# swesterfeld/audiowmark

Hardware: AMD Instinct MI355X
Metric: audio seconds watermarked+decoded per wall-second (xRT), 44.1 kHz stereo (higher is better)
Workload: dtype f32; 1 GPU; 60 min stereo 44.1 kHz white noise per GPU resident in HBM, add+get incl. payload decode, payload 0123456789abcdef0011223344556677, strength 10; parallelism=1 GPU, patterns=108, payload_matches=104, ranks_seen=1

## Files before the change

audiowmark_amd/binding.py:

```python
import ctypes as C
import os

import numpy as np

_HERE = os.path.dirname(os.path.abspath(__file__))
N_BANDS = 81
BLOCK_FRAMES = 2226
SOFT_BITS = 858


class AwmError(RuntimeError):
    pass


def library_path():
    return os.path.join(_HERE, "libawm_hip.so")




def _load_hip_runtime():
    candidates = []
    try:
        import torch
# ... 61 lines not shown
lib.awm_version.restype = C.c_char_p
lib.awm_ctx_stream.restype = C.c_void_p
lib.awm_search_approx_d.restype = C.c_long
lib.awm_set_params.argtypes = [C.c_double, C.c_int, C.c_int, C.c_int, C.c_double, C.c_int, C.c_double]
lib.awm_set_params.restype = None
lib.awm_ctx_create.argtypes = [C.c_int, C.POINTER(_vp)]
lib.awm_ctx_destroy.argtypes = [_vp]
lib.awm_ctx_destroy.restype = None
lib.awm_ctx_synchronize.argtypes = [_vp]
lib.awm_ctx_stream.argtypes = [_vp]
lib.awm_ctx_set_stream.argtypes = [_vp, _vp]
lib.awm_stft_d.argtypes = [_vp, _vp, C.c_size_t, C.c_int, C.c_size_t, C.c_size_t, C.c_size_t, _vp]
lib.awm_add_init_block_max_d.argtypes = [_vp, _vp, C.c_size_t]
lib.awm_add_mix_d.argtypes = [_vp, _vp, _vp, C.c_size_t, C.c_int, _vp, C.c_double, C.c_size_t, _vp, _vp, _vp,
                              C.c_size_t, C.c_size_t]
lib.awm_add_limit_d.argtypes = [_vp, _vp, C.c_size_t, C.c_int, C.c_size_t, _vp, C.c_size_t, C.c_size_t]
lib.awm_add_d.argtypes = [_vp, _vp, _vp, C.c_size_t, C.c_int, _vp, C.c_double, C.c_int]
lib.awm_sync_fft_d.argtypes = [_vp, _vp, C.c_size_t, C.c_int, C.c_size_t, C.c_size_t, _vp, C.c_size_t, C.c_size_t, _vp, _vp]
lib.awm_sync_search_d.argtypes = [_vp, _vp, _vp, C.c_size_t, C.c_int, C.c_int, C.c_size_t, _vp, _vp, _vp]
lib.awm_search_approx_d.argtypes = [_vp, _vp, _vp, C.c_size_t, C.c_int, C.c_int, C.c_size_t, _vp, _vp, _vp]
lib.awm_block_soft_bits_d.argtypes = [_vp, _vp, _vp, C.c_size_t, C.c_int, _vp, C.c_size_t, _vp, _vp]
lib.awm_viterbi_decode.argtypes = [_vp, C.c_int, _vp, C.c_size_t, C.c_size_t, _vp, _vp]
lib.awm_add_watermark_d.argtypes = [_vp, _vp, C.c_char_p, _vp, _vp, C.c_size_t, C.c_int, C.c_int]
lib.awm_get_watermark_d.argtypes = [_vp, _vp, _vp, C.c_size_t, C.c_int, C.c_size_t, _vp]
lib.awm_add_get_watermark_d.argtypes = [_vp, _vp, C.c_char_p, _vp, _vp, C.c_size_t, C.c_int, C.c_int, C.c_size_t, _vp]
lib.awm_resample_frames.argtypes = [_vp, C.c_size_t, C.c_int, C.c_int]
lib.awm_resample_frames.restype = C.c_size_t
lib.awm_resample_d.argtypes = [_vp, _vp, C.c_size_t, C.c_int, C.c_int, C.c_int, _vp, C.c_size_t]
lib.awm_add_watermark_payloads_d.argtypes = [_vp, _vp, _vp, C.c_size_t, _vp, _vp, C.c_size_t, C.c_int, C.c_int]
lib.awm_debug_set_add_payloads_fused.argtypes = [C.c_int]
lib.awm_debug_set_add_payloads_fused.restype = None
lib.awm_debug_add_payloads_fused_in_use.argtypes = []
lib.awm_debug_add_payloads_fused_in_use.restype = C.c_int
lib.awm_debug_add_payloads_tile.argtypes = []
lib.awm_debug_add_payloads_tile.restype = C.c_int
lib.awm_add_watermark_batch_d.argtypes = [_vp, _vp, C.c_char_p, C.c_size_t, _vp, _vp, _vp, C.c_int]
lib.awm_get_watermark_batch_d.argtypes = [_vp, _vp, C.c_size_t, _vp, _vp, C.c_int, C.c_int, C.c_size_t, _vp, _vp]
lib.awm_add_watermark_batch_keys_d.argtypes = [_vp, _vp, C.c_char_p, C.c_size_t, _vp, _vp, _vp, C.c_int]
lib.awm_get_watermark_batch_keys_d.argtypes = [_vp, _vp, C.c_size_t, _vp, _vp, C.c_int, C.c_int, C.c_size_t, _vp, _vp]
lib.awm_decode_chunk_d.argtypes = [_vp, _vp, _vp, C.c_size_t, C.c_int, C.c_int, C.c_size_t, _vp]
lib.awm_tab_up_down.argtypes = [_vp, C.c_int, C.c_int, _vp, _vp]
lib.awm_tab_bit_pos.argtypes = [_vp, _vp]
lib.awm_tab_mix_entries.argtypes = [_vp, _vp]
lib.awm_tab_bit_order.argtypes = [_vp, C.c_size_t, _vp]
lib.awm_tab_frame_mod.argtypes = [_vp, C.c_char_p, _vp]
lib.awm_tab_sync_bits.argtypes = [_vp, C.c_int, _vp]
lib.awm_tab_window.argtypes = [C.c_size_t, _vp]
lib.awm_tab_synth_window.argtypes = [_vp]
lib.awm_conv_encode.argtypes = [C.c_int, _vp, C.c_size_t, _vp]
lib.awm_test_gen_noise.argtypes = [_vp, C.c_size_t, _vp]


class RawFormat(C.Structure):
    _fields_ = [("n_channels", C.c_int), ("sample_rate", C.c_int), ("bit_depth", C.c_int), ("encoding", C.c_int), ("big_endian", C.c_int)]


lib.awm_add_watermark_file.argtypes = [_vp, _vp, C.c_char_p, C.c_char_p, C.c_char_p, C.POINTER(RawFormat), C.POINTER(RawFormat)]
lib.awm_add_stream_watermark_file.argtypes = [_vp, _vp, C.c_char_p, C.c_char_p, C.c_char_p, C.POINTER(RawFormat), C.POINTER(RawFormat), C.c_size_t]
lib.awm_add_stream_create_at.argtypes = [_vp, _vp, C.c_char_p, C.c_int, C.c_size_t, C.c_size_t, C.POINTER(_vp)]
lib.awm_debug_sync_db_sliding_d.argtypes = [_vp, _vp, C.c_size_t, C.c_int, _vp, C.c_size_t, C.c_int, C.c_int, _vp]
lib.awm_get_watermark_file.argtypes = [_vp, _vp, C.c_char_p, C.POINTER(RawFormat), C.c_size_t, _vp]
lib.awm_add_get_watermark_file.argtypes = [_vp, _vp, C.c_char_p, C.c_char_p, C.c_char_p, C.POINTER(RawFormat), C.POINTER(RawFormat), C.c_size_t, _vp]
lib.awm_add_stream_create.argtypes = [_vp, _vp, C.c_char_p, C.c_int, C.c_size_t, C.POINTER(_vp)]
lib.awm_add_stream_destroy.argtypes = [_vp]
lib.awm_add_stream_destroy.restype = None
lib.awm_add_stream_input.argtypes = [_vp]
# ... 862 lines not shown
```

audiowmark_amd/csrc/hip/kernels.hh:

```
#pragma once
#include <hip/hip_runtime.h>
#include <cstddef>
#include <cstdint>

#if defined(__HIP_DEVICE_COMPILE__) && !defined(__gfx950__)
#error "audiowmark_amd's HIP kernels are written for gfx950 (MI355X) only"
#endif

namespace awmk {

struct DevTables
{
  const float2 *tw512;
  const float2 *tw1024;
  const float  *window;
  const float  *synth;
  const double2 *slide;
  const double2 *tw512d;
  const float2 *slide32;
};

hipError_t launch_stft_full (hipStream_t st, const DevTables& t, const float *pcm, int n_channels,
                             long long start_index, long long hop, long long frame_count, float2 *out);

// ... 86 lines not shown
struct SyncDbArgs
{
  const float *pcm;
  long long    n_frames;
  int          n_channels;
  int          per_channel;
  long long    base0, base_stride;
  const long long *stream_base;
  int          count0;
  const int   *stream_count;
  long long    n_streams;
  long long    hop;
  float       *out;
  long long    out_stream_stride;
  long long    ld;
  char        *have;
  long long    have_stream_stride;
  long long    first, last;
  int          tile_frames;
  int          xcd_interleave = 0;
  const int           *row_perm = nullptr;
  const unsigned char *band_pos = nullptr;
  int                  rows_per_plane = 0;
  float               *tail = nullptr;
  long long            tail_stream_stride = 0;
  int                  tables_per_slice = 0;
  int                  streams_per_slice = 0;
  long long            slice_stride = 0;
  const long long     *stream_range = nullptr;
  const int           *range_index = nullptr;
  int                  range_div = 1;
  int                  silent_frames_are_zero = 0;
  int                  skip_unread_silent_tiles = 0;
};
hipError_t launch_sync_db (hipStream_t st, const DevTables& t, const SyncDbArgs& a);
hipError_t launch_sync_db_sliding (hipStream_t st, const DevTables& t, const SyncDbArgs& a);
bool sliding_rows_have_tail (int n_channels);

struct SyncTableDev
{
  const int *packed;
  int        rows_per_bit;
  const unsigned *chains = nullptr;
  long long       chains_slice_stride = 0;
  int             planes_per_slice = 1;
  const int      *row_frames = nullptr;
};
void pack_scan_chains (const int *packed, int rows_per_bit, unsigned *out );
struct SyncScanArgs
{
  const float *db;
  const char  *have;
  int          have_is_run = 0;
  long long    plane_stride;
  long long    have_plane_stride;
  long long    row_stride, band_stride, have_row_stride;
  long long    n_lanes;
  const int   *lane_count;
  long long    n_planes;
  double       min_delta;
  double      *quality;
  long long    q_stride;
  SyncTableDev table;
};
hipError_t launch_sync_scan (hipStream_t st, const SyncScanArgs& a);
hipError_t launch_sync_scan_window (hipStream_t st, const SyncScanArgs& a, int total_frames);

struct GatheredScanArgs
// ... 18 lines not shown
};
constexpr size_t GATHERED_SCRATCH_BYTES_PER_PLANE = 18 * 128 * 4;
hipError_t launch_sync_scan_gathered (hipStream_t st, const GatheredScanArgs& a);

hipError_t launch_local_mean (hipStream_t st, const double *q, long long q_stride, long long n_start_frames,
                              double *raw_sorted, double *local_mean, int n_slices = 1);

struct PeakOut { long long p; double raw, mean; };
hipError_t launch_peak_select (hipStream_t st, const double *raw_sorted, const double *local_mean, long long n, double threshold,
                               unsigned int *count, PeakOut *out, unsigned int cap);
hipError_t launch_peak_select_slices (hipStream_t st, const double *raw_sorted, const double *local_mean, long long n, double threshold,
                                      unsigned int *count, int count_stride, PeakOut *out, unsigned int cap, int n_slices);

hipError_t launch_peak_topk (hipStream_t st, const PeakOut *in, const unsigned int *count, unsigned int cap, PeakOut *out, int k, int n_slices);
hipError_t launch_peak_topk_lists (hipStream_t st, const PeakOut *in, const unsigned int *count, int count_stride, unsigned int cap,
                                   PeakOut *out, int k, int n_slices, int n_lists);

struct SoftBitsArgs
{
  const float   *db;
  long long      block_stride, ld;
  int            n_channels;
  const int16_t *mix_frame;
  const uint8_t *mix_up, *mix_down;
  int            n_data_frames;
  int            frames_per_bit;
  int            block_frames;
  long long      n_blocks;
  float         *out;
  const int     *block_slice = nullptr;
  const long long *block_base = nullptr;
  const long long *stream_range = nullptr;
  const int       *range_index = nullptr;
};
hipError_t launch_soft_bits (hipStream_t st, const SoftBitsArgs& a);

struct SoftJobDev
{
  int       mode;
  int       n_src, src_off;
  int       len;
  int       norm0, norm1;
  long long out_off;
  int       order_off;
  int       pad;
};
struct SoftPrepArgs
{
  const float      *raw;
  int               n_bits;
  const int        *inv_order;
  const SoftJobDev *jobs;
  const int2       *src;
  long long         n_jobs;
  int               hard;
  float            *out;
};
hipError_t launch_soft_prep (hipStream_t st, const SoftPrepArgs& a);

hipError_t launch_viterbi (hipStream_t st, const float *const soft[3], const long long n_blocks[3], long long n_steps,
                           unsigned char *const decisions_ws[3], int *const bits_out[3], float *const error_out[3], unsigned int *sync_ws);
size_t viterbi_workspace_bytes (long long coded_len, int rate, long long n_blocks);
bool viterbi_steps_supported (long long n_steps);
size_t viterbi_sync_bytes (long long n_blocks);
double probe_dependent_launch_us (hipStream_t st);
const char *viterbi_form_description();
// ... 103 lines not shown
```

audiowmark_amd/csrc/hip/kernels.hip:

```cpp
#include "kernels.hh"
#include "awm_fft.hip.h"
#include <cstdlib>
#include <algorithm>
#include <type_traits>

namespace awmk {

constexpr int NB = 81;
constexpr int MIN_BAND = 20;
constexpr int WAVES = 4;

typedef const int __attribute__ ((address_space (4))) *const_int_ptr;

__device__ __forceinline__ void
load_shared_tables (const DevTables& t, float2 *s_tw, float *s_win, float2 *s_twb)
{
  fft512_load_twiddles (t.tw512, s_tw);
  for (int i = threadIdx.x; i < 1024; i += blockDim.x)
    s_win[i] = t.window[i];
  if (s_twb)
    for (int i = threadIdx.x; i < NB; i += blockDim.x)
      s_twb[i] = t.tw1024[MIN_BAND + i];
}


__device__ __forceinline__ void
fetch_stereo (const float *pcm, long long idx, int avail, int lane, float (&l)[16], float (&r)[16])
{
  const float *p = pcm + idx * 2;
  if (avail >= 1024 && ((reinterpret_cast<uintptr_t> (p) & 15) == 0))
    {
      const float4 *p4 = reinterpret_cast<const float4 *> (p);
#pragma unroll
      for (int j = 0; j < 8; j++)
        {
          const float4 v = p4[lane + 64 * j];
          l[2 * j] = v.x; r[2 * j] = v.y; l[2 * j + 1] = v.z; r[2 * j + 1] = v.w;
// ... 1604 lines not shown

hipError_t
launch_mix_max (hipStream_t st, const float *orig, const float *wm, float *out, long long n_frames, int n_channels,
                unsigned int *block_max, long long n_blocks, int limiter_block)
{
  const long long n_values = n_frames * n_channels;
  if (n_values <= 0)
    return hipSuccess;
  if ((long long) limiter_block * n_channels < MIX_RUN)
    return hipErrorInvalidValue;
  hipLaunchKernelGGL (mix_max_kernel, dim3 (unsigned ((n_values + MIX_RUN - 1) / MIX_RUN)), dim3 (256), 0, st, orig, wm, out, n_values,
                      n_channels, block_max, n_blocks, limiter_block);
  return hipGetLastError();
}

__global__ void
fill_u32_kernel (unsigned int *p, unsigned int v, size_t n)
{
  const size_t i = (size_t) blockIdx.x * blockDim.x + threadIdx.x;
  if (i < n)
    p[i] = v;
}
hipError_t
launch_fill_u32 (hipStream_t st, unsigned int *p, unsigned int v, size_t n)
{
  if (!n)
    return hipSuccess;
  hipLaunchKernelGGL (fill_u32_kernel, dim3 (unsigned ((n + 255) / 256)), dim3 (256), 0, st, p, v, n);
  return hipGetLastError();
}


__device__ __forceinline__ long long
sync_stream_base (const SyncDbArgs& a, long long stream)
{
  if (a.stream_base)
    return a.stream_base[stream];
  if (a.streams_per_slice > 0)
    return a.base0 + (stream % a.streams_per_slice) * a.base_stride + (stream / a.streams_per_slice) * a.slice_stride;
  return a.base0 + stream * a.base_stride;
}

__device__ __forceinline__ void
sync_stream_range (const SyncDbArgs& a, long long stream, long long& first, long long& last)
{
  first = a.first;
  last = a.last;
  if (a.stream_range)
    {
      const long long g = stream / a.range_div;
      const long long slice = a.range_index ? a.range_index[g] : g;
      first = a.stream_range[2 * slice];
      last = a.stream_range[2 * slice + 1];
      if (first < 0)
        first = last = 0x7fffffffffffffffLL;
    }
}


template<int CV, bool SPLIT, int TLD> __global__ void __launch_bounds__ (64 * WAVES)
sync_db_kernel (DevTables t, SyncDbArgs a)
{
  constexpr int TILE_LD = TLD, TILE_MAX = TLD - 1, SPLIT_COLS = TILE_MAX / 2;
  __shared__ float2 s_tw[512];
  __shared__ float  s_win[1024];
  __shared__ float2 s_twb[NB];
  __shared__ float2 s_x[WAVES][XBUF_ELEMS];
  __shared__ float  s_tile[NB * TILE_LD];
  __shared__ char   s_have[TILE_MAX];
  const int lane = threadIdx.x & 63, wave = threadIdx.x >> 6;
  if (a.silent_frames_are_zero && a.skip_unread_silent_tiles)
    {
      long long stream = blockIdx.y, tile_idx = blockIdx.x;
      if (a.xcd_interleave)
        {
          const long long j = blockIdx.x >> 3;
          stream = j % a.n_streams;
          tile_idx = (j / a.n_streams) * 8 + (blockIdx.x & 7);
        }
      const long long base = sync_stream_base (a, stream);
      const int count = a.stream_count ? a.stream_count[stream] : a.count0;
      long long sil_first, sil_last;
      sync_stream_range (a, stream, sil_first, sil_last);
      const long long tile0 = tile_idx * a.tile_frames;
      if (tile0 >= count)
        return;
      const long long n_here = (count - tile0) < a.tile_frames ? count - tile0 : a.tile_frames;
      const long long idx_before = base + (tile0 - 2) * a.hop, idx_after = base + (tile0 + n_here + 1) * a.hop;
      const int C = a.n_channels;
      if ((idx_after + 1024) * C < sil_first || idx_before * C > sil_last)
        return;
    }
  load_shared_tables (t, s_tw, s_win, s_twb);
  __syncthreads();

  long long stream = blockIdx.y, tile_idx = blockIdx.x;
  if (a.xcd_interleave)
    {
      const long long j = blockIdx.x >> 3;
      stream = j % a.n_streams;
      tile_idx = (j / a.n_streams) * 8 + (blockIdx.x & 7);
    }
  const int plane_ch = blockIdx.z;
  const long long base = sync_stream_base (a, stream);
  const int count = a.stream_count ? a.stream_count[stream] : a.count0;
  long long sil_first, sil_last;
  sync_stream_range (a, stream, sil_first, sil_last);
  const int TF = a.tile_frames;
  const long long tile0 = tile_idx * TF;
  if (tile0 >= count)
    return;
  const int C = a.n_channels;
  float2 *xbuf = s_x[wave];
  const int n_here = (count - tile0) < TF ? int (count - tile0) : TF;

  for (int ff = wave; ff < n_here; ff += WAVES)
    {
      const long long idx = base + (tile0 + ff) * a.hop;
      const long long f_first = idx * C, f_last = (idx + 1024) * C;
      const bool outside = idx < 0 || idx + 1024 > a.n_frames;
      const bool skip = (f_last < sil_first) || (f_first > sil_last) || outside;
      float acc0 = 0.f, acc1 = 0.f;
      float split0 = 0.f, split1 = 0.f;
      if (!skip)
        {
          if (CV == 2)
            {
              float in[2][16];
              fetch_stereo (a.pcm, idx, 1024, lane, in[0], in[1]);
              float2 za[8], zb[8];
              window_pack (in[0], s_win, lane, za);
              window_pack (in[1], s_win, lane, zb);
              fft512_forward2 (za, zb, xbuf, s_tw, lane);
              const int k0 = MIN_BAND + lane, k1 = MIN_BAND + 64 + lane;
              const bool second = lane < NB - 64;
              float2 pa[4], pb[4];
              lds_st (&xbuf[0 * 64 + lane], za[0]);
              lds_st (&xbuf[1 * 64 + lane], za[1]);
              lds_st (&xbuf[6 * 64 + lane], za[6]);
              lds_st (&xbuf[7 * 64 + lane], za[7]);
              wave_sync();
              pa[0] = lds_ld (&xbuf[zpos (k0)]);
              pa[1] = lds_ld (&xbuf[zpos (512 - k0)]);
              pa[2] = lds_ld (&xbuf[zpos (second ? k1 : k0)]);
              pa[3] = lds_ld (&xbuf[zpos (512 - (second ? k1 : k0))]);
              wave_sync();
              lds_st (&xbuf[0 * 64 + lane], zb[0]);
              lds_st (&xbuf[1 * 64 + lane], zb[1]);
// ... 52 lines not shown
          const float zero_db = db_from_complex (make_float2 (0.f, 0.f));
          const int n_ch = CV == 2 ? 2 : (a.per_channel ? 1 : C);
          for (int c = 0; c < n_ch; c++)
            {
              if (SPLIT && c == 1)
                {
                  split0 = acc0;
                  split1 = acc1;
                  acc0 = acc1 = 0.f;
                }
              acc0 = __fadd_rn (acc0, zero_db);
              acc1 = __fadd_rn (acc1, zero_db);
            }
        }
      if (SPLIT)
        {
          s_tile[lane * TILE_LD + ff] = split0;
          s_tile[lane * TILE_LD + SPLIT_COLS + ff] = acc0;
          if (lane < NB - 64)
            {
              s_tile[(64 + lane) * TILE_LD + ff] = split1;
              s_tile[(64 + lane) * TILE_LD + SPLIT_COLS + ff] = acc1;
            }
        }
      else
        {
          s_tile[lane * TILE_LD + ff] = acc0;
          if (lane < NB - 64)
            s_tile[(64 + lane) * TILE_LD + ff] = acc1;
        }
      if (lane == 0)
        s_have[ff] = skip ? 0 : 1;
    }
  __syncthreads();
  if (SPLIT)
    {
      for (int p = 0; p < 2; p++)
        {
          float *out = a.out + stream * a.out_stream_stride + (long long) p * NB * a.ld + tile0;
          for (int i = threadIdx.x; i < NB * n_here; i += blockDim.x)
            {
              const int band = i / n_here, ff = i - band * n_here;
              out[band * a.ld + ff] = s_tile[band * TILE_LD + p * SPLIT_COLS + ff];
            }
        }
    }
  else
    {
      const long long plane = a.per_channel ? plane_ch : 0;
      float *out = a.out + stream * a.out_stream_stride + plane * NB * a.ld + tile0;
      for (int i = threadIdx.x; i < NB * n_here; i += blockDim.x)
        {
          const int band = i / n_here, ff = i - band * n_here;
          out[band * a.ld + ff] = s_tile[band * TILE_LD + ff];
        }
    }
  if (a.have && plane_ch == 0)
    for (int i = threadIdx.x; i < n_here; i += blockDim.x)
      a.have[stream * a.have_stream_stride + tile0 + i] = s_have[i];
}

hipError_t
launch_sync_db (hipStream_t st, const DevTables& t, const SyncDbArgs& a)
{
  if (a.n_streams <= 0 || a.tile_frames <= 0 || a.tile_frames > 72)
    return a.n_streams <= 0 ? hipSuccess : hipErrorInvalidValue;
  int max_count = a.count0;
  if (max_count <= 0)
    return hipSuccess;
  const unsigned tiles = unsigned ((max_count + a.tile_frames - 1) / a.tile_frames);
  if (a.n_streams > 65535LL * 1)
    {
      SyncDbArgs b = a;
      long long done = 0;
      while (done < a.n_streams)
        {
          const long long n = (a.n_streams - done) > 65535 ? 65535 : (a.n_streams - done);
          b.n_streams = n;
          b.base0 = a.base0 + done * a.base_stride;
          b.stream_base = a.stream_base ? a.stream_base + done : nullptr;
          b.stream_count = a.stream_count ? a.stream_count + done : nullptr;
          b.out = a.out + done * a.out_stream_stride;
          b.have = a.have ? a.have + done * a.have_stream_stride : nullptr;
          hipError_t e = launch_sync_db (st, t, b);
          if (e != hipSuccess)
            return e;
          done += n;
        }
      return hipSuccess;
    }
  const bool small = a.tile_frames <= 32;
  if (a.n_channels == 2 && a.per_channel)
    {
      SyncDbArgs b = a;
      b.tile_frames = 16;
      const unsigned split_tiles = unsigned ((max_count + b.tile_frames - 1) / b.tile_frames);
      hipLaunchKernelGGL ((sync_db_kernel<2, true, 33>), dim3 (split_tiles, unsigned (a.n_streams), 1), dim3 (64 * WAVES), 0, st, t, b);
      return hipGetLastError();
    }
  const unsigned planes = a.per_channel ? unsigned (a.n_channels) : 1u;
  dim3 grid (tiles, unsigned (a.n_streams), planes);
  SyncDbArgs b = a;
  if (!a.stream_base && !a.stream_count && a.n_streams >= 2 && a.n_streams <= 8 && planes == 1)
    {
      b.xcd_interleave = 1;
      grid = dim3 (unsigned (((tiles + 7) / 8) * 8 * a.n_streams), 1, 1);
    }
  if (a.n_channels == 2 && !a.per_channel)
    {
      if (small)
        hipLaunchKernelGGL ((sync_db_kernel<2, false, 33>), grid, dim3 (64 * WAVES), 0, st, t, b);
      else
        hipLaunchKernelGGL ((sync_db_kernel<2, false, 73>), grid, dim3 (64 * WAVES), 0, st, t, b);
    }
  else
    {
      if (small)
        hipLaunchKernelGGL ((sync_db_kernel<1, false, 33>), grid, dim3 (64 * WAVES), 0, st, t, b);
      else
        hipLaunchKernelGGL ((sync_db_kernel<1, false, 73>), grid, dim3 (64 * WAVES), 0, st, t, b);
    }
  return hipGetLastError();
}

constexpr int SL_TILE = 16;

__device__ __forceinline__ double
dpp_from_lower_lane (double v)
{
  const int lo = __builtin_amdgcn_update_dpp (0, __double2loint (v), 0x138, 0xf, 0xf, true);
  const int hi = __builtin_amdgcn_update_dpp (0, __double2hiint (v), 0x138, 0xf, 0xf, true);
  return __hiloint2double (hi, lo);
}
__device__ __forceinline__ double
dpp_from_upper_lane (double v)
{
  const int lo = __builtin_amdgcn_update_dpp (0, __double2loint (v), 0x130, 0xf, 0xf, true);
  const int hi = __builtin_amdgcn_update_dpp (0, __double2hiint (v), 0x130, 0xf, 0xf, true);
  return __hiloint2double (hi, lo);
}

__device__ __forceinline__ long long
wave_uniform (long long v)
{
  const int lo = __builtin_amdgcn_readfirstlane (int (v)), hi = __builtin_amdgcn_readfirstlane (int (v >> 32));
  return (long long) (((unsigned long long) (unsigned int) hi << 32) | (unsigned int) lo);
}

typedef __attribute__ ((address_space (1))) float global_float;
__device__ __forceinline__ global_float *
uniform_global (const float *p)
{
  return (global_float *) (unsigned long long) wave_uniform ((long long) (unsigned long long) p);
}

template<int CV> __global__ void __launch_bounds__ (64 * WAVES) __attribute__ ((amdgpu_waves_per_eu (3, 3)))
sync_db_sliding_kernel (DevTables t, SyncDbArgs a)
{
  constexpr int SCRATCH_FLOATS = XBUF_ELEMS * 4 > NB * SL_TILE ? XBUF_ELEMS * 4 : NB * SL_TILE;
  __shared__ __attribute__ ((aligned (16))) float s_scratch[WAVES][SCRATCH_FLOATS];
  __shared__ unsigned char s_pos[WAVES][NB + 3];
  __shared__ __attribute__ ((aligned (16))) double s_delta[WAVES][SL_TILE * 8 * CV];
  __shared__ int s_nzd[WAVES][SL_TILE * CV];
  __shared__ int s_x0[WAVES][SL_TILE * CV];
  {
    const int w = threadIdx.x >> 6, l = threadIdx.x & 63;
    const long long s = (long long) blockIdx.x * WAVES + w;
    const long long tslice = (a.tables_per_slice && s < a.n_streams) ? (a.range_index ? a.range_index[s / a.range_div] : s / a.range_div) : 0;
    for (int b = l; b < NB; b += 64)
      s_pos[w][b] = (a.band_pos && s < a.n_streams) ? a.band_pos[(tslice * a.rows_per_plane + s % a.rows_per_plane) * NB + b] : (unsigned char) b;
  }
  __syncthreads();

  const int lane = threadIdx.x & 63, wave = threadIdx.x >> 6;
  const long long stream = (long long) blockIdx.x * WAVES + wave;
  if (stream >= a.n_streams)
    return;
  const long long perm_slice = a.tables_per_slice ? (a.range_index ? a.range_index[stream / a.range_div] : stream / a.range_div) : 0;
  const long long out_slot = wave_uniform (a.row_perm ? (stream / a.rows_per_plane) * a.rows_per_plane
// ... 1136 lines not shown
  const int n_bits = a.n_data_frames / a.frames_per_bit;
  if (bit >= n_bits)
    return;
  const float *db = a.db + blk * a.block_stride;
  const int C = a.n_channels;
  const long long mix0 = a.block_slice ? (long long) a.block_slice[blk] * a.n_data_frames * 30 : 0;
  const int16_t *mix_frame = a.mix_frame + mix0;
  const uint8_t *mix_up = a.mix_up + mix0, *mix_down = a.mix_down + mix0;
  double umag = 0, dmag = 0;
  for (int f = bit * a.frames_per_bit; f < (bit + 1) * a.frames_per_bit; f++)
    for (int ch = 0; ch < C; ch++)
      {
        const float *plane = db + (long long) ch * NB * a.ld;
        for (int j = 0; j < 30; j++)
          {
            const int b = f * 30 + j;
            const int frame = mix_frame[b];
            const int next = frame + 1 < a.block_frames ? frame + 1 : frame - 1;
            const int prev = frame - 1 >= 0 ? frame - 1 : frame + 1;
            const float *pu = plane + (long long) (mix_up[b] - MIN_BAND) * a.ld;
            const float *pd = plane + (long long) (mix_down[b] - MIN_BAND) * a.ld;
            umag += pu[frame];
            umag -= double (__fadd_rn (pu[prev], pu[next])) * 0.5;
            dmag += pd[frame];
            dmag -= double (__fadd_rn (pd[prev], pd[next])) * 0.5;
          }
      }
  a.out[blk * n_bits + bit] = float (umag - dmag);
}

constexpr int SB_WAVES = 4;
constexpr int SB_BPW = 4;
constexpr int SB_MAX_ITEMS = 256;

__global__ void __launch_bounds__ (64 * SB_WAVES)
soft_bits_wave_kernel (SoftBitsArgs a, int groups_per_block)
{
  extern __shared__ __attribute__ ((aligned (16))) float4 s_item_dyn[];
  const int lane = threadIdx.x & 63, wave = threadIdx.x >> 6;
  const long long slot = blockIdx.x >> 3;
  const long long blk = (slot / groups_per_block) * 8 + (blockIdx.x & 7);
  const int group = int (slot % groups_per_block);
  if (blk >= a.n_blocks)
    return;
  const int n_bits = a.n_data_frames / a.frames_per_bit;
  const int bit0 = (group * SB_WAVES + wave) * SB_BPW;
  if (bit0 >= n_bits)
    return;
  const float *db = a.db + blk * a.block_stride;
  const int C = a.n_channels;
  const long long mix0 = a.block_slice ? (long long) a.block_slice[blk] * a.n_data_frames * 30 : 0;
  const int16_t *mix_frame = a.mix_frame + mix0;
  const uint8_t *mix_up = a.mix_up + mix0, *mix_down = a.mix_down + mix0;
  const int n_items = a.frames_per_bit * C * 30;
  float4 *items = s_item_dyn + (size_t) wave * SB_BPW * n_items;
  const int n_here = min (SB_BPW, n_bits - bit0);
  int live_lo = 0, live_hi = 0x7fffffff;
  if (a.stream_range)
    {
      const long long sl = a.range_index[blk];
      const long long first = a.stream_range[2 * sl], last = a.stream_range[2 * sl + 1];
      live_lo = a.block_frames;
      live_hi = -1;
      if (first >= 0)
        {
          const long long base = a.block_base[blk];
          const long long lo_num = (first + C - 1) / C - 1024 - base, hi_num = last / C - base;
          const long long lo = lo_num <= 0 ? 0 : (lo_num + 1023) / 1024, hi = hi_num < 0 ? -1 : hi_num / 1024;
          live_lo = int (lo < a.block_frames ? lo : a.block_frames);
          live_hi = int (hi < a.block_frames ? hi : a.block_frames - 1);
        }
    }
  const float zero_db = db_from_complex (make_float2 (0.f, 0.f));
  for (int i = lane; i < n_items; i += 64)
#pragma unroll
  for (int q = 0; q < SB_BPW; q++)
    {
      const int e = q * n_items + i;
      const int bit = bit0 + min (q, n_here - 1);
      const int fi = i / (C * 30), ch = (i / 30) % C, j = i % 30;
      const int b = (bit * a.frames_per_bit + fi) * 30 + j;
      const int frame = mix_frame[b];
      const int next = frame + 1 < a.block_frames ? frame + 1 : frame - 1;
      const int prev = frame - 1 >= 0 ? frame - 1 : frame + 1;
      if (max (frame, max (prev, next)) < live_lo || min (frame, min (prev, next)) > live_hi)
        {
          items[e] = make_float4 (zero_db, __fadd_rn (zero_db, zero_db), zero_db, __fadd_rn (zero_db, zero_db));
          continue;
        }
      const float *plane = db + (long long) ch * NB * a.ld;
      const float *pu = plane + (long long) (mix_up[b] - MIN_BAND) * a.ld;
      const float *pd = plane + (long long) (mix_down[b] - MIN_BAND) * a.ld;
      items[e] = make_float4 (pu[frame], __fadd_rn (pu[prev], pu[next]), pd[frame], __fadd_rn (pd[prev], pd[next]));
    }
  wave_sync();
  if (lane < n_here)
    {
      const float4 *mine = items + lane * n_items;
      double umag = 0, dmag = 0;
      for (int i = 0; i < n_items; i++)
        {
          const float4 t = mine[i];
          umag = __dadd_rn (umag, double (t.x));
          umag = __dsub_rn (umag, __dmul_rn (double (t.y), 0.5));
          dmag = __dadd_rn (dmag, double (t.z));
          dmag = __dsub_rn (dmag, __dmul_rn (double (t.w), 0.5));
        }
      a.out[blk * n_bits + bit0 + lane] = float (__dsub_rn (umag, dmag));
    }
}

int g_soft_bits_generic = 0;
extern "C" void awm_debug_set_soft_bits_generic (int on) { g_soft_bits_generic = on; }

hipError_t
launch_soft_bits (hipStream_t st, const SoftBitsArgs& a)
{
  if (a.n_blocks <= 0)
    return hipSuccess;
  const int n_bits = a.n_data_frames / a.frames_per_bit;
  if (!g_soft_bits_generic && a.frames_per_bit * a.n_channels * 30 <= SB_MAX_ITEMS)
    {
      const int groups = (n_bits + SB_WAVES * SB_BPW - 1) / (SB_WAVES * SB_BPW);
      const long long rounds = (a.n_blocks + 7) / 8;
      const long long wgs = rounds * groups * 8;
      const size_t lds = size_t (SB_WAVES) * SB_BPW * (a.frames_per_bit * a.n_channels * 30) * sizeof (float4);
      if (wgs < (1LL << 31))
        {
          hipLaunchKernelGGL (soft_bits_wave_kernel, dim3 (unsigned (wgs)), dim3 (64 * SB_WAVES), lds, st, a, groups);
          return hipGetLastError();
        }
    }
  const dim3 grid (unsigned ((n_bits + 127) / 128), unsigned (a.n_blocks));
  hipLaunchKernelGGL (soft_bits_kernel, grid, dim3 (128), 0, st, a);
  return hipGetLastError();
}

__global__ void __launch_bounds__ (256)
nonzero_range_kernel (const float *data, long long n_values, unsigned long long *result)
{
  const long long stride = (long long) gridDim.x * blockDim.x;
  unsigned long long first = ~0ULL, last = 0;
  for (long long i = (long long) blockIdx.x * blockDim.x + threadIdx.x; i < n_values; i += stride)
    if (data[i] != 0.f)
      {
        if ((unsigned long long) i < first) first = i;
        if ((unsigned long long) i + 1 > last) last = i + 1;
      }
  for (int o = 32; o > 0; o >>= 1)
    {
      const unsigned long long f = __shfl_xor (first, o), l = __shfl_xor (last, o);
      first = f < first ? f : first;
// ... 594 lines not shown
```

include/awm_hip.h:

```cpp
#ifndef AWM_HIP_H
#define AWM_HIP_H

#include <stddef.h>
#include <stdint.h>

#ifdef __cplusplus
extern "C" {
#endif

#define AWM_ERR_GENERIC    (-1)
#define AWM_ERR_NO_DEVICE  (-2)
#define AWM_ERR_ARG        (-3)
#define AWM_ERR_HIP        (-4)
#define AWM_ERR_IO         (-5)

#define AWM_FRAME_SIZE      1024
#define AWM_N_BANDS         81
#define AWM_BLOCK_FRAMES    2226
#define AWM_SOFT_BITS       858

typedef struct awm_ctx awm_ctx;

const char *awm_last_error (void);
const char *awm_version (void);
// ... 178 lines not shown

int awm_ctx_set_helpers (awm_ctx *ctx, awm_ctx *const *helpers, int n_helpers);

void awm_set_speed_params (int detect_speed, int detect_speed_patient, double try_speed, double test_speed);
size_t awm_resample_ratio_frames (size_t n_frames, int n_channels, int rate, double ratio, double max_in_seconds);
int awm_resample_ratio_d (awm_ctx *ctx, const float *pcm_in_d, size_t n_frames, int n_channels, int rate, double ratio,
                          double max_in_seconds, float *out_d, size_t n_out_frames);
int awm_detect_speed_d (awm_ctx *ctx, const uint8_t key[16], const float *pcm_d, size_t n_frames, int n_channels, int rate,
                        int patient, double *speed_out, double *quality_out);
int awm_speed_clip_location_d (awm_ctx *ctx, const uint8_t key[16], const float *pcm_d, size_t n_frames, int n_channels, int rate,
                               double seconds, int candidates, double *location);
int awm_speed_mags_d (awm_ctx *ctx, const uint8_t key[16], const float *pcm_d, size_t n_frames, int n_channels, int rate,
                      double clip_location, double center, double seconds, size_t max_rows, float *out);
int awm_speed_scan_d (awm_ctx *ctx, const uint8_t key[16], const float *pcm_d, size_t n_frames, int n_channels, int rate,
                      double clip_location, double seconds, double step, int n_steps, int n_center_steps,
                      const double *speeds, int n_speeds, size_t max_out, double *out_speed, double *out_quality);

int    awm_speed_select_n_best (double *speed, double *quality, int count, int n);
double awm_speed_smooth_best (const double *speed, const double *quality, int count, double step, double distance);
size_t awm_speed_clip_positions (const uint8_t key[16], size_t n_values, size_t max_out, uint64_t *positions);
int    awm_speed_clip_candidates (const uint8_t key[16], const float *hashed_values, size_t n, int candidates, double *locations);

void awm_debug_set_viterbi_super (int on);
void awm_debug_set_viterbi_persistent (int on);
double awm_debug_dependent_launch_us (void);
int  awm_debug_viterbi_one_launch_in_use (void);
void awm_debug_set_sliding3 (int on);
void awm_debug_set_refine_form (int form);
int  awm_debug_refine_form (void);
void awm_debug_set_k4s_ablate (int flags);
int  awm_debug_sync_db_sliding_d (awm_ctx *ctx, const float *pcm_d, size_t n_frames, int n_channels, const long long *base_d, size_t n_streams,
                                  int count, int ld, float *out_d);
void awm_debug_set_soft_bits_generic (int on);
void awm_debug_set_scan_generic (int on);
int  awm_debug_scan_generic_launches (void);
void awm_debug_set_chunk_stagger (int mode);
void awm_debug_set_resample_phase (int on);
void awm_debug_set_get_overlap (int on);
void awm_debug_set_speed_compare_wide (int on);
void awm_debug_set_speed_compare_fold (int on);
void awm_debug_set_resample_var_mode (int mode);
void awm_debug_set_speed_overlap (int on);
int  awm_debug_frame_mod_tables_d (awm_ctx *ctx, const uint8_t *keys, size_t n_keys, const char *payload_hex, int8_t *tables_out);
int  awm_debug_clip_key_tables_check_d (awm_ctx *ctx, const uint8_t *keys, size_t n_keys, long long mismatch_out[9]);
void awm_debug_set_key_tables_on_device (int on);
void awm_debug_set_merge_decodes (int on);
void awm_debug_set_add_batched (int on);
void awm_debug_set_add_slab_mb (int mb);
void awm_debug_set_add_payloads_fused (int on);
int  awm_debug_add_payloads_fused_in_use (void);
void awm_debug_set_payloads_file_tile (int frames1024);
int  awm_debug_add_payloads_tile (void);
void awm_debug_set_fft_pair (int on);
void awm_debug_set_clip_poison (int on);
void awm_debug_set_clip_pad_margin (int frames);
void awm_debug_set_staged_threads (int n);
void awm_debug_clip_key_timing (double us_out[3]);
double awm_debug_time_group_key_tables (int n_keys, int threads);
void awm_debug_set_group_fallback (int on);
void awm_debug_alloc_stats (long *dev_allocs, double *dev_ms, long *pinned_allocs, double *pinned_ms);
void awm_debug_file_timing (double ms_out[8]);
void awm_debug_set_io_flags (int flags);

void awm_set_io_threads (int n);

void awm_set_quiet (int quiet);
// ... 33 lines not shown
```

Before: 740,800 xRT.

## Make sync_db kernel persistent with balanced tile splitting and vectorize soft-bit row loads

Turns the small-tile sync_db kernel into a persistent grid sized to resident workgroups, each looping over a balanced range of frame units (with optional sub-tile units chosen to minimize tail imbalance). Shared tables are loaded once per workgroup instead of once per tile, and output stores use a column-major mapping per band. It also sets a waves-per-EU occupancy hint and makes soft_bits load three adjacent floats per row in one access. The intent is to cut per-tile launch and table-load overhead and wave-quantization tail, at the cost of more complex indexing and reliance on occupancy queries.

New measurement: 719,000 xRT. 0.971x the previous value.

```diff
diff --git a/audiowmark_amd/binding.py b/audiowmark_amd/binding.py
--- a/audiowmark_amd/binding.py
+++ b/audiowmark_amd/binding.py
@@ -117,6 +117,12 @@
 lib.awm_debug_set_add_payloads_fused.restype = None
 lib.awm_debug_add_payloads_fused_in_use.argtypes = []
 lib.awm_debug_add_payloads_fused_in_use.restype = C.c_int
+lib.awm_debug_set_sync_db_split.argtypes = [C.c_int]
+lib.awm_debug_set_sync_db_split.restype = None
+lib.awm_debug_set_sync_db_resident_workgroups.argtypes = [C.c_int]
+lib.awm_debug_set_sync_db_resident_workgroups.restype = None
+lib.awm_debug_sync_db_resident_workgroups.argtypes = [C.c_int]
+lib.awm_debug_sync_db_resident_workgroups.restype = C.c_int
 lib.awm_debug_add_payloads_tile.argtypes = []
 lib.awm_debug_add_payloads_tile.restype = C.c_int
 lib.awm_add_watermark_batch_d.argtypes = [_vp, _vp, C.c_char_p, C.c_size_t, _vp, _vp, _vp, C.c_int]
diff --git a/audiowmark_amd/csrc/hip/kernels.hh b/audiowmark_amd/csrc/hip/kernels.hh
--- a/audiowmark_amd/csrc/hip/kernels.hh
+++ b/audiowmark_amd/csrc/hip/kernels.hh
@@ -142,8 +142,12 @@
   int                  range_div = 1;
   int                  silent_frames_are_zero = 0;
   int                  skip_unread_silent_tiles = 0;
+  int                  split_mode = 0;
+  int                  split_unit = 0;
+  long long            split_units = 0;
 };
 hipError_t launch_sync_db (hipStream_t st, const DevTables& t, const SyncDbArgs& a);
+int sync_db_resident_workgroups (int inst);
 hipError_t launch_sync_db_sliding (hipStream_t st, const DevTables& t, const SyncDbArgs& a);
 bool sliding_rows_have_tail (int n_channels);
 
@@ -228,6 +232,7 @@
   const long long *block_base = nullptr;
   const long long *stream_range = nullptr;
   const int       *range_index = nullptr;
+  int              row_loads = 0;
 };
 hipError_t launch_soft_bits (hipStream_t st, const SoftBitsArgs& a);
 
diff --git a/audiowmark_amd/csrc/hip/kernels.hip b/audiowmark_amd/csrc/hip/kernels.hip
--- a/audiowmark_amd/csrc/hip/kernels.hip
+++ b/audiowmark_amd/csrc/hip/kernels.hip
@@ -3,6 +3,7 @@
 #include <cstdlib>
 #include <algorithm>
 #include <type_traits>
+#include <atomic>
 
 namespace awmk {
 
@@ -1673,6 +1674,13 @@
 
 
 __device__ __forceinline__ long long
+wave_uniform (long long v)
+{
+  const int lo = __builtin_amdgcn_readfirstlane (int (v)), hi = __builtin_amdgcn_readfirstlane (int (v >> 32));
+  return (long long) (((unsigned long long) (unsigned int) hi << 32) | (unsigned int) lo);
+}
+
+__device__ __forceinline__ long long
 sync_stream_base (const SyncDbArgs& a, long long stream)
 {
   if (a.stream_base)
@@ -1699,62 +1707,13 @@
 }
 
 
-template<int CV, bool SPLIT, int TLD> __global__ void __launch_bounds__ (64 * WAVES)
-sync_db_kernel (DevTables t, SyncDbArgs a)
-{
-  constexpr int TILE_LD = TLD, TILE_MAX = TLD - 1, SPLIT_COLS = TILE_MAX / 2;
-  __shared__ float2 s_tw[512];
-  __shared__ float  s_win[1024];
-  __shared__ float2 s_twb[NB];
-  __shared__ float2 s_x[WAVES][XBUF_ELEMS];
-  __shared__ float  s_tile[NB * TILE_LD];
-  __shared__ char   s_have[TILE_MAX];
+template<int CV, bool SPLIT, int TLD> __device__ __forceinline__ void
+sync_db_tile_frames (const SyncDbArgs& a, long long base, long long tile0, int n_here, long long sil_first, long long sil_last, int plane_ch,
+                     const float2 *s_tw, const float *s_win, const float2 *s_twb, float2 *xbuf, float *s_tile, char *s_have)
+{
+  constexpr int TILE_LD = TLD, SPLIT_COLS = (TLD - 1) / 2;
   const int lane = threadIdx.x & 63, wave = threadIdx.x >> 6;
-  if (a.silent_frames_are_zero && a.skip_unread_silent_tiles)
-    {
-      long long stream = blockIdx.y, tile_idx = blockIdx.x;
-      if (a.xcd_interleave)
-        {
-          const long long j = blockIdx.x >> 3;
-          stream = j % a.n_streams;
-          tile_idx = (j / a.n_streams) * 8 + (blockIdx.x & 7);
-        }
-      const long long base = sync_stream_base (a, stream);
-      const int count = a.stream_count ? a.stream_count[stream] : a.count0;
-      long long sil_first, sil_last;
-      sync_stream_range (a, stream, sil_first, sil_last);
-      const long long tile0 = tile_idx * a.tile_frames;
-      if (tile0 >= count)
-        return;
-      const long long n_here = (count - tile0) < a.tile_frames ? count - tile0 : a.tile_frames;
-      const long long idx_before = base + (tile0 - 2) * a.hop, idx_after = base + (tile0 + n_here + 1) * a.hop;
-      const int C = a.n_channels;
-      if ((idx_after + 1024) * C < sil_first || idx_before * C > sil_last)
-        return;
-    }
-  load_shared_tables (t, s_tw, s_win, s_twb);
-  __syncthreads();
-
-  long long stream = blockIdx.y, tile_idx = blockIdx.x;
-  if (a.xcd_interleave)
-    {
-      const long long j = blockIdx.x >> 3;
-      stream = j % a.n_streams;
-      tile_idx = (j / a.n_streams) * 8 + (blockIdx.x & 7);
-    }
-  const int plane_ch = blockIdx.z;
-  const long long base = sync_stream_base (a, stream);
-  const int count = a.stream_count ? a.stream_count[stream] : a.count0;
-  long long sil_first, sil_last;
-  sync_stream_range (a, stream, sil_first, sil_last);
-  const int TF = a.tile_frames;
-  const long long tile0 = tile_idx * TF;
-  if (tile0 >= count)
-    return;
   const int C = a.n_channels;
-  float2 *xbuf = s_x[wave];
-  const int n_here = (count - tile0) < TF ? int (count - tile0) : TF;
-
   for (int ff = wave; ff < n_here; ff += WAVES)
     {
       const long long idx = base + (tile0 + ff) * a.hop;
@@ -1873,32 +1832,223 @@
       if (lane == 0)
         s_have[ff] = skip ? 0 : 1;
     }
-  __syncthreads();
-  if (SPLIT)
-    {
-      for (int p = 0; p < 2; p++)
-        {
-          float *out = a.out + stream * a.out_stream_stride + (long long) p * NB * a.ld + tile0;
-          for (int i = threadIdx.x; i < NB * n_here; i += blockDim.x)
-            {
-              const int band = i / n_here, ff = i - band * n_here;
-              out[band * a.ld + ff] = s_tile[band * TILE_LD + p * SPLIT_COLS + ff];
-            }
-        }
+}
+
+template<int CV, bool SPLIT, int TLD> __global__ void __launch_bounds__ (64 * WAVES)
+__attribute__ ((amdgpu_waves_per_eu (TLD == 33 ? 4 : 3, TLD == 33 ? 4 : 3)))
+sync_db_kernel (DevTables t, SyncDbArgs a)
+{
+  constexpr int TILE_LD = TLD, TILE_MAX = TLD - 1;
+  __shared__ float2 s_tw[512];
+  __shared__ float  s_win[1024];
+  __shared__ float2 s_twb[NB];
+  __shared__ float2 s_x[WAVES][XBUF_ELEMS];
+  __shared__ float  s_tile[NB * TILE_LD];
+  __shared__ char   s_have[TILE_MAX];
+  const int wave = threadIdx.x >> 6;
+  const int TF = a.tile_frames, unit = a.split_unit;
+  const long long ups = a.split_units, n_units = a.n_streams * ups;
+  int plane_ch = 0;
+  long long lo, hi, adv = n_units;
+  if (a.split_mode == 0)
+    {
+      long long stream = blockIdx.y, tile_idx = blockIdx.x;
+      if (a.xcd_interleave)
+        {
+          const long long j = blockIdx.x >> 3;
+          stream = j % a.n_streams;
+          tile_idx = (j / a.n_streams) * 8 + (blockIdx.x & 7);
+        }
+      plane_ch = blockIdx.z;
+      lo = stream * ups + tile_idx;
+      hi = tile_idx < ups ? lo + 1 : lo;
+    }
+  else if (a.split_mode == 2)
+    {
+      lo = blockIdx.x;
+      hi = lo + 1;
+      adv = gridDim.x;
+    }
+  else if (a.xcd_interleave)
+    {
+      const long long j = blockIdx.x >> 3, slots = gridDim.x / a.n_streams;
+      const long long stream = j % a.n_streams, slot = (j / a.n_streams) * 8 + (blockIdx.x & 7);
+      lo = stream * ups + slot * ups / slots;
+      hi = stream * ups + (slot + 1) * ups / slots;
     }
   else
     {
-      const long long plane = a.per_channel ? plane_ch : 0;
-      float *out = a.out + stream * a.out_stream_stride + plane * NB * a.ld + tile0;
-      for (int i = threadIdx.x; i < NB * n_here; i += blockDim.x)
-        {
-          const int band = i / n_here, ff = i - band * n_here;
-          out[band * a.ld + ff] = s_tile[band * TILE_LD + ff];
-        }
-    }
-  if (a.have && plane_ch == 0)
-    for (int i = threadIdx.x; i < n_here; i += blockDim.x)
-      a.have[stream * a.have_stream_stride + tile0 + i] = s_have[i];
+      lo = blockIdx.x * n_units / gridDim.x;
+      hi = (blockIdx.x + 1) * n_units / gridDim.x;
+    }
+  lo = wave_uniform (lo);
+  hi = wave_uniform (hi);
+  adv = wave_uniform (adv);
+  const int C = a.n_channels;
+  long long s_lo = 0, s_hi = 0;
+  long long stream = 0, base = 0, sil_first = 0, sil_last = 0;
+  int count = 0;
+  bool tables_loaded = false;
+  for (; lo < n_units; lo += adv, hi += adv)
+    for (long long cur = lo; cur < hi;)
+      {
+        if (cur < s_lo || cur >= s_hi)
+          {
+            stream = wave_uniform (cur / ups);
+            s_lo = stream * ups;
+            s_hi = s_lo + ups;
+            base = wave_uniform (sync_stream_base (a, stream));
+            count = __builtin_amdgcn_readfirstlane (a.stream_count ? a.stream_count[stream] : a.count0);
+            sync_stream_range (a, stream, sil_first, sil_last);
+            sil_first = wave_uniform (sil_first);
+            sil_last = wave_uniform (sil_last);
+          }
+        const unsigned run_end = unsigned ((hi < s_hi ? hi : s_hi) - s_lo) * unsigned (unit);
+        const unsigned p0 = unsigned (cur - s_lo) * unsigned (unit);
+        unsigned p1 = (p0 / unsigned (TF) + 1) * unsigned (TF);
+        p1 = p1 < run_end ? p1 : run_end;
+        const unsigned next_unit = __builtin_amdgcn_readfirstlane (p1 / unsigned (unit));
+        p1 = __builtin_amdgcn_readfirstlane (p1);
+        cur = s_lo + next_unit;
+        const long long tile0 = p0, tile1 = p1;
+        if (tile0 >= count)
+          continue;
+        const int n_here = int ((tile1 < count ? tile1 : count) - tile0);
+        if (a.silent_frames_are_zero && a.skip_unread_silent_tiles)
+          {
+            const long long idx_before = base + (tile0 - 2) * a.hop, idx_after = base + (tile0 + n_here + 1) * a.hop;
+            if ((idx_after + 1024) * C < sil_first || idx_before * C > sil_last)
+              continue;
+          }
+        if (!tables_loaded)
+          {
+            load_shared_tables (t, s_tw, s_win, s_twb);
+            __syncthreads();
+            tables_loaded = true;
+          }
+        sync_db_tile_frames<CV, SPLIT, TLD> (a, base, tile0, n_here, sil_first, sil_last, plane_ch, s_tw, s_win, s_twb, s_x[wave], s_tile, s_have);
+        __syncthreads();
+        if (TLD == 33)
+          {
+            const int col = threadIdx.x & 31;
+            const int ff = SPLIT ? col & 15 : col;
+            const long long plane = SPLIT ? col >> 4 : (a.per_channel ? plane_ch : 0);
+            const int band0 = threadIdx.x >> 5;
+            float *out = a.out + stream * a.out_stream_stride + (plane * NB + band0) * a.ld + tile0 + ff;
+            if (ff < n_here)
+#pragma unroll 1
+              for (int band = band0; band < NB; band += 64 * WAVES / 32, out += 64 * WAVES / 32 * a.ld)
+                *out = s_tile[band * TILE_LD + col];
+          }
+        else
+          {
+            const long long plane = a.per_channel ? plane_ch : 0;
+            float *out = a.out + stream * a.out_stream_stride + plane * NB * a.ld + tile0;
+            for (int i = threadIdx.x; i < NB * n_here; i += blockDim.x)
+              {
+                const int band = i / n_here, ff = i - band * n_here;
+                out[band * a.ld + ff] = s_tile[band * TILE_LD + ff];
+              }
+          }
+        if (a.have && plane_ch == 0)
+          for (int i = threadIdx.x; i < n_here; i += blockDim.x)
+            a.have[stream * a.have_stream_stride + tile0 + i] = s_have[i];
+        __syncthreads();
+      }
+}
+
+int g_sync_db_split = 1;
+extern "C" void awm_debug_set_sync_db_split (int on) { g_sync_db_split = on; }
+int g_sync_db_resident = 0;
+extern "C" void awm_debug_set_sync_db_resident_workgroups (int g) { g_sync_db_resident = g > 0 ? g : 0; }
+
+int
+sync_db_resident_workgroups (int inst)
+{
+  constexpr int MAX_DEVICES = 64;
+  static std::atomic<int> cache[MAX_DEVICES][3];
+  if (g_sync_db_resident)
+    return g_sync_db_resident / 8 * 8;
+  int dev = -1;
+  if (inst < 0 || inst > 2 || hipGetDevice (&dev) != hipSuccess || dev < 0 || dev >= MAX_DEVICES)
+    {
+      (void) hipGetLastError();
+      return 0;
+    }
+  int g = cache[dev][inst].load (std::memory_order_relaxed);
+  if (!g)
+    {
+      int per_cu = 0, cus = 0;
+      hipError_t e;
+      if (inst == 0)
+        e = hipOccupancyMaxActiveBlocksPerMultiprocessor (&per_cu, sync_db_kernel<1, false, 33>, 64 * WAVES, 0);
+      else if (inst == 1)
+        e = hipOccupancyMaxActiveBlocksPerMultiprocessor (&per_cu, sync_db_kernel<2, false, 33>, 64 * WAVES, 0);
+      else
+        e = hipOccupancyMaxActiveBlocksPerMultiprocessor (&per_cu, sync_db_kernel<2, true, 33>, 64 * WAVES, 0);
+      if (e == hipSuccess)
+        e = hipDeviceGetAttribute (&cus, hipDeviceAttributeMultiprocessorCount, dev);
+      g = -1;
+      if (e == hipSuccess && per_cu > 0 && cus > 0)
+        g = std::max (per_cu * cus / 8 * 8, -1);
+      else
+        (void) hipGetLastError();
+      if (g == 0)
+        g = -1;
+      cache[dev][inst].store (g, std::memory_order_relaxed);
+    }
+  return g > 0 ? g : 0;
+}
+extern "C" int awm_debug_sync_db_resident_workgroups (int inst) { return sync_db_resident_workgroups (inst); }
+
+static void
+sync_db_plan_tiles (SyncDbArgs& b, int max_count)
+{
+  b.split_mode = 0;
+  b.split_unit = b.tile_frames;
+  b.split_units = (max_count + b.tile_frames - 1) / b.tile_frames;
+}
+
+static void
+sync_db_plan_split (SyncDbArgs& b, int inst, int max_count, dim3& grid)
+{
+  sync_db_plan_tiles (b, max_count);
+  if (!g_sync_db_split || b.stream_count || max_count > (1 << 30))
+    return;
+  long long G = sync_db_resident_workgroups (inst);
+  if (b.xcd_interleave)
+    G -= G % (8 * b.n_streams);
+  if (G <= 0 || b.n_streams * b.split_units <= G)
+    return;
+  grid = dim3 (unsigned (G), 1, 1);
+  if (b.skip_unread_silent_tiles)
+    {
+      b.split_mode = 2;
+      return;
+    }
+  const long long W = b.xcd_interleave ? G / b.n_streams : G;
+  int best_u = 0;
+  double best_imb = 0;
+  for (int div = 1; div <= 4; div *= 2)
+    {
+      const int u = b.tile_frames / div;
+      if (b.tile_frames % div || u % WAVES)
+        break;
+      const long long ups = (max_count + u - 1) / u, n = b.xcd_interleave ? ups : b.n_streams * ups;
+      const double imb = double ((n + W - 1) / W * W) / double (n) - 1.0;
+      if (!best_u || imb < best_imb)
+        {
+          best_u = u;
+          best_imb = imb;
+        }
+      if (imb <= 0.05)
+        break;
+    }
+  if (!best_u)
+    best_u = b.tile_frames;
+  b.split_mode = 1;
+  b.split_unit = best_u;
+  b.split_units = (max_count + best_u - 1) / best_u;
 }
 
 hipError_t
@@ -1936,12 +2086,15 @@
       SyncDbArgs b = a;
       b.tile_frames = 16;
       const unsigned split_tiles = unsigned ((max_count + b.tile_frames - 1) / b.tile_frames);
-      hipLaunchKernelGGL ((sync_db_kernel<2, true, 33>), dim3 (split_tiles, unsigned (a.n_streams), 1), dim3 (64 * WAVES), 0, st, t, b);
+      dim3 grid (split_tiles, unsigned (a.n_streams), 1);
+      sync_db_plan_split (b, 2, max_count, grid);
+      hipLaunchKernelGGL ((sync_db_kernel<2, true, 33>), grid, dim3 (64 * WAVES), 0, st, t, b);
       return hipGetLastError();
     }
   const unsigned planes = a.per_channel ? unsigned (a.n_channels) : 1u;
   dim3 grid (tiles, unsigned (a.n_streams), planes);
   SyncDbArgs b = a;
+  sync_db_plan_tiles (b, max_count);
   if (!a.stream_base && !a.stream_count && a.n_streams >= 2 && a.n_streams <= 8 && planes == 1)
     {
       b.xcd_interleave = 1;
@@ -1950,14 +2103,21 @@
   if (a.n_channels == 2 && !a.per_channel)
     {
       if (small)
-        hipLaunchKernelGGL ((sync_db_kernel<2, false, 33>), grid, dim3 (64 * WAVES), 0, st, t, b);
+        {
+          sync_db_plan_split (b, 1, max_count, grid);
+          hipLaunchKernelGGL ((sync_db_kernel<2, false, 33>), grid, dim3 (64 * WAVES), 0, st, t, b);
+        }
       else
         hipLaunchKernelGGL ((sync_db_kernel<2, false, 73>), grid, dim3 (64 * WAVES), 0, st, t, b);
     }
   else
     {
       if (small)
-        hipLaunchKernelGGL ((sync_db_kernel<1, false, 33>), grid, dim3 (64 * WAVES), 0, st, t, b);
+        {
+          if (planes == 1)
+            sync_db_plan_split (b, 0, max_count, grid);
+          hipLaunchKernelGGL ((sync_db_kernel<1, false, 33>), grid, dim3 (64 * WAVES), 0, st, t, b);
+        }
       else
         hipLaunchKernelGGL ((sync_db_kernel<1, false, 73>), grid, dim3 (64 * WAVES), 0, st, t, b);
     }
@@ -1979,13 +2139,6 @@
   const int lo = __builtin_amdgcn_update_dpp (0, __double2loint (v), 0x130, 0xf, 0xf, true);
   const int hi = __builtin_amdgcn_update_dpp (0, __double2hiint (v), 0x130, 0xf, 0xf, true);
   return __hiloint2double (hi, lo);
-}
-
-__device__ __forceinline__ long long
-wave_uniform (long long v)
-{
-  const int lo = __builtin_amdgcn_readfirstlane (int (v)), hi = __builtin_amdgcn_readfirstlane (int (v >> 32));
-  return (long long) (((unsigned long long) (unsigned int) hi << 32) | (unsigned int) lo);
 }
 
 typedef __attribute__ ((address_space (1))) float global_float;
@@ -3188,6 +3341,7 @@
 constexpr int SB_WAVES = 4;
 constexpr int SB_BPW = 4;
 constexpr int SB_MAX_ITEMS = 256;
+struct __attribute__ ((packed, aligned (4))) SoftBitsRow3 { float v[3]; };
 
 __global__ void __launch_bounds__ (64 * SB_WAVES)
 soft_bits_wave_kernel (SoftBitsArgs a, int groups_per_block)
@@ -3247,6 +3401,20 @@
       const float *plane = db + (long long) ch * NB * a.ld;
       const float *pu = plane + (long long) (mix_up[b] - MIN_BAND) * a.ld;
       const float *pd = plane + (long long) (mix_down[b] - MIN_BAND) * a.ld;
+      if (a.row_loads)
+        {
+          const int mid = min (max (frame, 1), a.block_frames - 2);
+          const SoftBitsRow3 u3 = *reinterpret_cast<const SoftBitsRow3 *> (pu + mid - 1);
+          const SoftBitsRow3 d3 = *reinterpret_cast<const SoftBitsRow3 *> (pd + mid - 1);
+          const bool at_first = frame < mid, at_last = frame > mid;
+          const float u_frame = at_first ? u3.v[0] : (at_last ? u3.v[2] : u3.v[1]);
+          const float d_frame = at_first ? d3.v[0] : (at_last ? d3.v[2] : d3.v[1]);
+          const bool edge = at_first || at_last;
+          const float u_prev = edge ? u3.v[1] : u3.v[0], u_next = edge ? u3.v[1] : u3.v[2];
+          const float d_prev = edge ? d3.v[1] : d3.v[0], d_next = edge ? d3.v[1] : d3.v[2];
+          items[e] = make_float4 (u_frame, __fadd_rn (u_prev, u_next), d_frame, __fadd_rn (d_prev, d_next));
+          continue;
+        }
       items[e] = make_float4 (pu[frame], __fadd_rn (pu[prev], pu[next]), pd[frame], __fadd_rn (pd[prev], pd[next]));
     }
   wave_sync();
@@ -3270,10 +3438,12 @@
 extern "C" void awm_debug_set_soft_bits_generic (int on) { g_soft_bits_generic = on; }
 
 hipError_t
-launch_soft_bits (hipStream_t st, const SoftBitsArgs& a)
-{
-  if (a.n_blocks <= 0)
+launch_soft_bits (hipStream_t st, const SoftBitsArgs& a0)
+{
+  if (a0.n_blocks <= 0)
     return hipSuccess;
+  SoftBitsArgs a = a0;
+  a.row_loads = g_sync_db_split && a.block_frames >= 3;
   const int n_bits = a.n_data_frames / a.frames_per_bit;
   if (!g_soft_bits_generic && a.frames_per_bit * a.n_channels * 30 <= SB_MAX_ITEMS)
     {
diff --git a/include/awm_hip.h b/include/awm_hip.h
--- a/include/awm_hip.h
+++ b/include/awm_hip.h
@@ -234,6 +234,9 @@
 int  awm_debug_sync_db_sliding_d (awm_ctx *ctx, const float *pcm_d, size_t n_frames, int n_channels, const long long *base_d, size_t n_streams,
                                   int count, int ld, float *out_d);
 void awm_debug_set_soft_bits_generic (int on);
+void awm_debug_set_sync_db_split (int on);
+int  awm_debug_sync_db_resident_workgroups (int inst);
+void awm_debug_set_sync_db_resident_workgroups (int g);
 void awm_debug_set_scan_generic (int on);
 int  awm_debug_scan_generic_launches (void);
 void awm_debug_set_chunk_stagger (int mode);
```
